# proycon/analiticcl

Hardware: AMD Instinct MI355X
Metric: scored (query,candidate) pairs/sec + queries/sec, 200k-lexicon, len≤16, 1/2/4/8 GPU (higher is better)
Workload: dtype u8

## Files before the change

analiticcl_amd/_lib.py:

```python
from __future__ import annotations

import ctypes as C
import os

HERE = os.path.dirname(os.path.abspath(__file__))
LIB_PATH = os.environ.get("ANX_LIB") or os.path.join(HERE, "libanx.so")

ANX_OK, ANX_EINVAL, ANX_EIO, ANX_ENOTBUILT, ANX_ENODEVICE, ANX_ELIMIT, ANX_EEMPTY = 0, -1, -2, -3, -4, -5, -6
ANX_NO_VIA = 0xFFFFFFFFFFFFFFFF
ABI_VERSION = 3


class AnxError(RuntimeError):
    def __init__(self, code: int, message: str):
        super().__init__(f"anx error {code}: {message}")
        self.code = code


class Weights(C.Structure):
    _fields_ = [("ld", C.c_double), ("lcs", C.c_double), ("prefix", C.c_double), ("suffix", C.c_double),
                ("casew", C.c_double)]


class Threshold(C.Structure):
# ... 185 lines not shown
        "anx_shutdown": (None, []),
        "anx_pipeline_new": (vp, [vp, C.c_int]),
        "anx_pipeline_submit_packed": (C.c_int, [vp, cp, C.c_size_t, C.c_size_t, C.POINTER(Params)]),
        "anx_pipeline_pending": (C.c_int, [vp]),
        "anx_pipeline_next": (C.c_int, [vp, C.POINTER(vp), C.POINTER(C.POINTER(C.c_uint32)), C.POINTER(C.c_size_t)]),
        "anx_pipeline_next_via": (C.c_int, [vp, C.POINTER(vp), C.POINTER(C.POINTER(C.c_uint32)), C.POINTER(C.POINTER(C.c_uint32)), C.POINTER(C.c_size_t)]),
        "anx_pipeline_free": (None, [vp]),
        "anx_debug_kernel_timer": (None, [C.c_int]),
        "anx_debug_kernel_time": (C.c_int, [cp, C.POINTER(C.c_double), C.POINTER(C.c_uint64)]),
        "anx_debug_length_split": (C.c_int, [vp, C.POINTER(C.c_char_p), C.c_size_t, C.POINTER(Params), C.c_int, vp, vp]),
        "anx_debug_signature": (C.c_int, [vp, cp, C.POINTER(C.c_uint64)]),
        "anx_debug_entries": (C.c_int, [vp, C.POINTER(C.POINTER(C.c_uint32)), C.POINTER(C.c_size_t)]),
        "anx_debug_adjacency": (C.c_int, [vp, C.c_int, C.c_uint64, vp, C.c_size_t, vp, C.POINTER(C.POINTER(C.c_uint32)), vp]),
        "anx_debug_adjacency_device": (C.c_int, [vp, vp, C.c_size_t, vp, C.POINTER(C.POINTER(C.c_uint32))]),
        "anx_debug_band_bound": (C.c_int, [C.c_int, vp, vp, vp, vp, C.c_size_t, C.c_int, C.c_int, vp]),
        "anx_batch_free": (None, [vp]),
        "anx_device_pool_trim": (None, [C.c_int]),
    }
    for name, (res, args) in sig.items():
        fn = getattr(L, name)
        fn.restype = res
        fn.argtypes = args
    _lib = L
    return L


EXPORTED = None


def set_switch(name: str, value) -> None:
# ... 21 lines not shown
```

analiticcl_amd/csrc/engine.h:

```cpp
#pragma once
#include <cstdint>
#include <string>
#include <vector>

#include "host_model.h"
#include "adjacency.h"

namespace anx {

struct DeviceLexicon;
struct Batch;

int device_count(std::string& err);
DeviceLexicon* lexicon_upload(const LexiconImage& img, const EncodeTables& et, const AdjIndex* adj, int device, std::string& err, int dev_closure = -1,
                              size_t dev_budget = 0, AdjIndex* dev_stats = nullptr);
void lexicon_free(DeviceLexicon*);
int debug_band_bound(int device, const uint8_t* q_rows, const uint8_t* c_rows, const uint8_t* lq, const uint8_t* lc, size_t n, int d, int form,
                     uint8_t* out, std::string& err);
void kernel_timer_enable(bool on);
bool kernel_timer_read(const char* name, double* total_ms, uint64_t* launches);
void device_pool_trim(int device);
void* stream_create(int device, std::string& err, bool high_priority = false);
void stream_destroy(int device, void* stream);
void* host_result_alloc(size_t bytes);
bool host_result_is_pinned(void* p);
void host_result_free(void* p);
void* thread_stream_begin(int device);
void thread_stream_end(int device, void* stream);
void encoder_stream_set_override(void* stream);
void host_result_cache_stats(uint64_t* hits, uint64_t* misses, uint64_t* miss_bytes);

Batch* batch_encode(const HostModel& m, const DeviceLexicon* dl, const char* const* utf8, size_t n,
                    const anx_params& p, std::string& err, int* code, bool keep_text = false);
// ... 124 lines not shown
```

analiticcl_amd/csrc/engine.hip:

```cpp
#include <hip/hip_runtime.h>

#include <algorithm>
#include <atomic>
#include <functional>
#include <chrono>
#include <cmath>
#include <cstdio>
#include <cstdlib>
#include <cstring>
#include <map>
#include <memory>
#include <mutex>
#include <unordered_map>
#include <numeric>
#include <thread>
#include <type_traits>

#include "engine_internal.h"

namespace anx {

#define HIP_TRY(expr)                                                                          \
  do {                                                                                         \
    hipError_t _e = (expr);                                                                    \
// ... 882 lines not shown
static void shells_destroy(int device) {
  DevPool& pl = pool_of(device);
  std::vector<BatchShell> drop;
  { std::lock_guard<std::mutex> g(pl.mu); drop.swap(pl.shells); }
  for (BatchShell& sh : drop) {
    for (auto& e : sh.ev) if (e) (void)hipEventDestroy(e);
    for (hipEvent_t e : {sh.ev_fs0, sh.ev_fs1, sh.ev_scan0, sh.ev_done, sh.ev_in}) if (e) (void)hipEventDestroy(e);
    if (sh.h_read) (void)hipHostFree(sh.h_read);
  }
}

static int encode_tail(Batch* b, std::string& err) {
  const size_t nq = b->nq;
  int rc;
  const size_t nblk = (nq + SCAN_TILE - 1) / SCAN_TILE + 2;
  if ((rc = dalloc(&b->counters, CTR_N, err)) || (rc = dalloc(&b->rctr, SCAN_REGIONS * RC_STRIDE, err)) || (rc = dalloc(&b->sctr, SCAN_REGIONS * RC_STRIDE, err)) || (rc = dalloc(&b->lctr, 3 * SCAN_REGIONS * RC_STRIDE, err)) || (rc = dalloc(&b->qexpand, nq, err)) || (rc = dalloc(&b->qsurv, nq, err)) ||
      (rc = dalloc(&b->soff, nq + 1, err)) || (rc = dalloc(&b->qcur, nq, err)) || (rc = dalloc(&b->qmaxfreq, nq, err)) ||
      (rc = dalloc(&b->scan_tmp, nblk, err)) || (rc = dalloc(&b->r_count, nq, err)) || (rc = dalloc(&b->r_off, nq + 1, err)))
    return rc;
  return shell_acquire(b, err);
}

Batch* batch_encode_spans(const HostModel& m, const DeviceLexicon* dl, const char* blob, size_t blob_bytes, const uint32_t* off, size_t n,
                          const anx_params& p, std::string& err, int* code, bool keep_text, bool blob_on_device, bool after_stream, void* src_stream) {
  *code = ANX_OK;
  if (blob_on_device && (off || switches().encode_host)) { err = "inputs in device memory need the device-side encoder and no host offsets"; *code = ANX_EINVAL; return nullptr; }
  if (!dl) { err = "model is not resident on a device (no HIP device / anx_model_to_device not called)"; *code = ANX_ENODEVICE; return nullptr; }
  if (hipSetDevice(dl->device) != hipSuccess) { err = "hipSetDevice failed"; *code = ANX_ENODEVICE; return nullptr; }
  if (n >= (1u << 27)) { err = "more than 2^27 inputs per batch"; *code = ANX_ELIMIT; return nullptr; }
  Batch* b = new Batch();
  b->device = dl->device;
  b->params = p;
  b->n_input = n;
  b->keep_text = keep_text;
// ... 54 lines not shown
  HostBuf<char> blob(part[nthreads] + 1);
  if (!blob.data()) { err = "out of memory"; *code = ANX_ELIMIT; return nullptr; }
  run_threads([&](unsigned t, size_t lo, size_t hi) {
    size_t pos = part[t];
    for (size_t i = lo; i < hi; ++i) {
      off[i] = (uint32_t)pos;
      if (lens[i]) memcpy(&blob[pos], utf8[i], lens[i]);
      blob[pos + lens[i]] = '\0';
      pos += (size_t)lens[i] + 1;
    }
  });
  off[n] = (uint32_t)part[nthreads];
  return batch_encode_spans(m, dl, blob.data(), blob.size(), off.data(), n, p, err, code, keep_text);
}

static int exclusive_scan(const uint32_t* in, uint32_t n, uint32_t* out, uint32_t* tmp, hipStream_t st, uint32_t* maxout = nullptr, uint32_t* copy = nullptr) {
  const uint32_t nb = (n + SCAN_TILE - 1) / SCAN_TILE;
  if (nb == 0) return hipMemsetAsync(out, 0, sizeof(uint32_t), st) == hipSuccess ? 0 : -1;
  hipLaunchKernelGGL(k_scan_local, dim3(nb), dim3(SCAN_THREADS), 0, st, in, n, out, tmp, maxout);
  hipLaunchKernelGGL(k_scan_sums, dim3(1), dim3(SCAN_THREADS), 0, st, tmp, nb);
  hipLaunchKernelGGL(k_scan_add, dim3(nb), dim3(SCAN_THREADS), 0, st, out, n, tmp, nb, copy);
  return 0;
}

namespace {
struct KTimerRec { std::string name; hipEvent_t e0 = nullptr, e1 = nullptr; int device = 0; bool closed = false; };
struct KTimer {
  std::mutex mu;
  std::atomic<bool> on{false};
  std::vector<KTimerRec> pending;
  uint32_t generation = 0;
  std::map<std::string, std::pair<double, uint64_t>> acc;
};
KTimer& ktimer() { static KTimer* t = new KTimer; return *t; }
void ktimer_resolve_locked(KTimer& t) {
  for (KTimerRec& r : t.pending) {
// ... 210 lines not shown
int Run::setup() {
  int rc;
  hints_apply(dl, b);
  if (b->raw_cap == 0 && b->hinted && (rc = ensure_raw(b, (size_t)b->prev_maxfill + (b->prev_maxfill >> 3) + 4096, err))) return rc;
  if (b->raw_cap == 0 && (rc = ensure_raw(b, (nq * (size_t)140 + (size_t)b->ntiles * SCAN_CHUNK) / SCAN_REGIONS / cap_div() + 4096, err)))
    return rc;
  region_cap = 1u << b->region_shift;
  fill_cap = b->prev_maxfill ? (uint32_t)std::min<size_t>(region_cap, (size_t)b->prev_maxfill + (b->prev_maxfill >> 3) + FS_BLK) : region_cap;
  b->fill_cap_launched = fill_cap;
  HIP_TRY(hipEventRecord(b->ev[0], st));
  return ANX_OK;
}

int Run::scan() {
  int rc;
  HIP_TRY(hipMemsetAsync(b->counters, 0, CTR_N * sizeof(uint32_t), st));
  HIP_TRY(hipMemsetAsync(b->rctr, 0, SCAN_REGIONS * RC_STRIDE * sizeof(uint32_t), st));
  if (b->ntiles == 0) { HIP_TRY(hipEventRecord(b->ev_scan0, st)); HIP_TRY(hipEventRecord(b->ev[5], st)); }
  if (b->ntiles) {
    ScanArgs A = scan_args_of(dl);
    A.tiles = b->d_tiles; A.ntiles = b->ntiles; A.q_bits = b->q_bits; A.q_cv = b->q_cv;
    A.chunk = SCAN_CHUNK;
    A.chunk_fused = switches().scan_chunk_fused ? (uint32_t)switches().scan_chunk_fused : SCAN_CHUNK_FUSED;
#ifdef ANX_DEBUG_SWITCHES
    { const char* e = getenv("ANX_SCAN_CHUNK"); const int v = e ? atoi(e) : 0; if (v >= 32 && v <= 1024) A.chunk = (uint32_t)v; }
#endif
    A.raw = b->raw; A.region_cap = region_cap; A.rctr = b->rctr; A.qexact = b->qexact; A.want_exact = stop;
    A.drop_len = (!stop && !b->keep_all_pairs) ? 1 : 0;
    A.q_rec = b->q_rec;
    A.fuse = (switches().fuse_prefilter && switches().prefilter && A.drop_len) ? 1 : 0;
    A.qpairs = nullptr;
    if (b->count_pairs) {
      if (!b->qpairs && (rc = dalloc(&b->qpairs, nq, err))) return rc;
      HIP_TRY(hipMemsetAsync(b->qpairs, 0, nq * sizeof(uint32_t), st));
      A.qpairs = b->qpairs;
    }
    A.dbg = 0;
#ifdef ANX_DEBUG_SWITCHES
    { const char* e = getenv("ANX_SCAN_DBG"); A.dbg = e ? atoi(e) : 0; }
#endif
    const uint32_t nsad = b->n_sad_tiles, nbits = A.ntiles - nsad, nadj = std::min(b->n_adj_tiles, nbits);
    with_nplanes(dl->nplanes, [&](auto np) { launch_scan<decltype(np)::value>(A, nadj, nbits, nsad, st, b->ev_scan0, b->ev[5]); });
  }
  HIP_TRY(hipMemcpyAsync(b->h_read + HR_RCTR, b->rctr, SCAN_REGIONS * RC_STRIDE * sizeof(uint32_t), hipMemcpyDeviceToHost, st));
  HIP_TRY(hipEventRecord(b->ev[1], st));
  b->n_raw = (uint32_t)(SCAN_REGIONS << b->region_shift);
  return ANX_OK;
}

int Run::score() {
  int rc;
  HIP_TRY(hipMemsetAsync(b->qsurv, 0, nq * sizeof(uint32_t), st));
  HIP_TRY(hipMemsetAsync(b->qmaxfreq, 0, nq * sizeof(uint32_t), st));
  if (dl->any_variants) HIP_TRY(hipMemsetAsync(b->qexpand, 0, nq * sizeof(uint32_t), st));
  ScorePlan plan = score_plan_of(m, dl, b->params.score_threshold, b->qw, b->dmax);
  ScoreArgs& sa = plan.sa;
#ifdef ANX_DEBUG_SWITCHES
  { const char* e = getenv("ANX_SCORE_DBG"); sa.dbg = e ? atoi(e) : 0; }
#endif
  sa.store_pairs = b->keep_all_pairs ? 1 : 0;
  if (sa.store_pairs && (rc = ensure_pair_outputs(b, err))) return rc;
  if (!plan.fits()) { err = "per-lane scoring state exceeds the LDS budget"; return ANX_ELIMIT; }
  const int fastD = plan.fastD;
  if ((rc = ensure_surv_records(b, b->prev_surv_fill ? (size_t)b->prev_surv_fill + (b->prev_surv_fill >> 3) + 256 : (size_t)fill_cap / 2 / cap_div() + 256, err))) return rc;
  so = SurvOut{b->surv, b->sctr, (uint32_t)b->surv_region_cap, nullptr, seg_capacity(dl, b)};
  so.seg = so.seg_cap ? b->sseg : nullptr;
  const bool need_lists = !fastD || plan.have_long_q || dl->max_len > 16;
  if (need_lists && (rc = ensure_slot_lists(b, b->prev_list_fill ? (size_t)b->prev_list_fill + (b->prev_list_fill >> 3) + 256 : (fastD ? (size_t)fill_cap / 2 : (size_t)fill_cap) / cap_div() + 256, err)))
    return rc;
  HIP_TRY(hipMemsetAsync(b->sctr, 0, SCAN_REGIONS * RC_STRIDE * sizeof(uint32_t), st));
  HIP_TRY(hipMemsetAsync(b->lctr, 0, 3 * SCAN_REGIONS * RC_STRIDE * sizeof(uint32_t), st));
  const SlotLists sl = slot_lists_of(b->list8, b->listg, b->listw, b->lctr, (uint32_t)b->list_cap);
  const PairArgs pa = pair_args_of(dl, b->raw, b->q_meta, b->q_rows, b->q_rec, b->p_score, b->p_meta, b->qmaxfreq, b->qsurv, b->qexpand);
  FilterArgs fa;
  fa.region_shift = b->region_shift; fa.rctr = b->rctr; fa.qexact = b->qexact; fa.stop = stop; fa.enable = plan.enable_filter;
  fa.use_nw8 = (plan.have_long_q || fastD > 0) ? 1 : 0; fa.counters = b->counters; fa.stat_ctr = b->sctr; fa.fill_cap = fill_cap; fa.blk = FS_BLK;
  const dim3 fgrid(((fill_cap + FS_BLK - 1) / FS_BLK) * SCAN_REGIONS);
  {
    FsCold* cold = reinterpret_cast<FsCold*>(reinterpret_cast<char*>(b->h_read) + HR_COLD_OFF);
    *cold = FsCold{sa, so, sl.l8, sl.lg, sl.lw};
    if (!b->d_cold && (rc = dalloc(reinterpret_cast<char**>(&b->d_cold), sizeof(FsCold), err))) return rc;
    HIP_TRY(hipMemcpyAsync(b->d_cold, cold, sizeof(FsCold), hipMemcpyHostToDevice, st));
  }
  HIP_TRY(hipEventRecord(b->ev_fs0, st));
  launch_filter_score(plan, fgrid, st, fa, pa, static_cast<const FsCold*>(b->d_cold));
  HIP_TRY(hipEventRecord(b->ev_fs1, st));
  if (need_lists) {
    const dim3 lgrid(LIST_P * SCAN_REGIONS);
    if (plan.split_wide && plan.enable_filter) hipLaunchKernelGGL(k_filter_wide, lgrid, dim3(256), 0, st, sl.lw, fa, pa, sa, fastD, sl.l8, sl.lg);
    if (fastD) launch_score_fast8(fastD, lgrid, st, sl.l8, pa, sa, so);
    hipLaunchKernelGGL(k_score_pairs, lgrid, dim3(plan.threads), plan.lds_bytes(), st, sl.lg, pa, sa, so);
  }
  HIP_TRY(hipEventRecord(b->ev[2], st));
  return ANX_OK;
}

int Run::compact_rank() {
  int rc;
  const RankArgs ra = rank_args_of(m, dl, b->params, b->conf_mode == 1 ? 0.0 : b->params.cutoff_threshold);
  exclusive_scan(b->qsurv, nq, b->soff, b->scan_tmp, st, nullptr, b->qcur);
  if (dl->any_variants) {
    uint32_t total_surv = 0;
    HIP_TRY(hipMemcpyAsync(&total_surv, b->soff + nq, sizeof(uint32_t), hipMemcpyDeviceToHost, st));
    HIP_TRY(hipMemcpyAsync(b->h_read + HR_SCTR, b->sctr, SCAN_REGIONS * RC_STRIDE * sizeof(uint32_t), hipMemcpyDeviceToHost, st));
    HIP_TRY(hipStreamSynchronize(st));
    uint32_t surv_fill = 0;
    for (uint32_t r = 0; r < SCAN_REGIONS; ++r) surv_fill = std::max(surv_fill, b->h_read[HR_SCTR + r * RC_STRIDE]);
    if ((size_t)surv_fill > b->surv_region_cap) {
      surv_fill = 0;
      HIP_TRY(hipMemsetAsync(b->counters + CTR_OVERFLOW, 0xFF, sizeof(uint32_t), st));
    }
    if ((rc = ensure_surv(b, (size_t)total_surv + (total_surv >> 2) + 1024, err))) return rc;
    if (surv_fill) {
      CompactArgs ca{m.have_freq ? 1 : 0, dl->any_variants};
      hipLaunchKernelGGL(k_compact, dim3(((surv_fill + 255) / 256) * SCAN_REGIONS), dim3(256), 0, st, b->surv, b->sctr,
                         (uint32_t)b->surv_region_cap, ca, b->qcur, dl->ent_rec, dl->ent_var_off, dl->var_target,
                         dl->var_target_freq, dl->var_score, b->c_rows);
    }
  } else if (b->surv_cap == 0 && (rc = ensure_surv(b, b->hint_rows ? b->hint_rows : (size_t)nq * 16 / cap_div() + 1024, err))) return rc;
  const uint32_t row_cap = (uint32_t)std::min<size_t>(b->surv_cap, 0xFFFFFFFFu);
  if (!dl->any_variants)
    hipLaunchKernelGGL(k_compact_grouped, dim3(COMPACT_P * SCAN_REGIONS), dim3(COMPACT_B), 0, st, b->surv, b->sctr,
                       (uint32_t)b->surv_region_cap, m.have_freq ? 1 : 0, b->qcur, dl->ent_rec, b->c_rows, b->soff + nq, row_cap,
                       b->counters + CTR_OVERFLOW);
  HIP_TRY(hipEventRecord(b->ev[3], st));
  if (b->conf_mode == 2 && (rc = conf_launch(m, dl, b, st, true, row_cap, err))) return rc;
  launch_rank(ra, st, nq, b->soff, b->c_rows, b->qmaxfreq, b->qexpand, b->t_key, b->r_rows, b->r_count, dl->any_variants ? 0xFFFFFFFFu : row_cap, b->counters + CTR_OVERFLOW,
              dl->any_variants ? SegRows{nullptr, 0u, nullptr} : SegRows{so.seg, so.seg_cap, dl->ent_rec});
  if (b->conf_mode == 1 && (rc = conf_launch(m, dl, b, st, false, row_cap, err))) return rc;
  exclusive_scan(b->r_count, nq, b->r_off, b->scan_tmp, st, b->counters + CTR_MAXROWS);
  HIP_TRY(hipEventRecord(b->ev[4], st));
  return ANX_OK;
}

int Run::readback() {
  HIP_TRY(hipMemcpyAsync(b->h_read + HR_SCTR, b->sctr, SCAN_REGIONS * RC_STRIDE * sizeof(uint32_t), hipMemcpyDeviceToHost, st));
  HIP_TRY(hipMemcpyAsync(b->h_read + HR_LCTR, b->lctr, 3 * SCAN_REGIONS * RC_STRIDE * sizeof(uint32_t), hipMemcpyDeviceToHost, st));
  HIP_TRY(hipMemcpyAsync(b->h_read + HR_CTR, b->counters, CTR_N * sizeof(uint32_t), hipMemcpyDeviceToHost, st));
  HIP_TRY(hipMemcpyAsync(b->h_read + HR_TOTAL_SURV, b->soff + nq, sizeof(uint32_t), hipMemcpyDeviceToHost, st));
  HIP_TRY(hipMemcpyAsync(b->h_read + HR_TOTAL_RESULTS, b->r_off + nq, sizeof(uint32_t), hipMemcpyDeviceToHost, st));
  b->h_read[HR_CONF] = b->h_read[HR_CONF + 1] = 0;
  if (b->conf_mode && b->cf_ctr) HIP_TRY(hipMemcpyAsync(b->h_read + HR_CONF, b->cf_ctr, 2 * sizeof(uint32_t), hipMemcpyDeviceToHost, st));
  HIP_TRY(hipEventRecord(b->ev_done, st));
  HIP_TRY(hipGetLastError());
  return ANX_OK;
}

static int batch_launch(const HostModel& m, const DeviceLexicon* dl, Batch* b, void* stream, std::string& err) {
  if (!dl) { err = "model is not resident on a device"; return ANX_ENODEVICE; }
  if (b->nq >= (1u << 27) || dl->nentries >= (1u << 26)) { err = "more than 2^27 queries per batch or 2^26 lexicon entries (32-bit record offsets, packed pair records)"; return ANX_ELIMIT; }
  HIP_TRY(hipSetDevice(dl->device));
  if (b->launched) {
    HIP_TRY(hipEventSynchronize(b->ev_done));
    b->launched = false;
  }
  b->last_stream = stream;
  b->ran = false;
// ... 431 lines not shown
  HIP_TRY(hipSetDevice(b->device));
  off.assign(b->n_input + 1, 0u);
  HIP_TRY(hipMemcpy(off.data(), b->d_textoff, (b->n_input + 1) * sizeof(uint32_t), hipMemcpyDeviceToHost));
  text.assign(b->n_input ? (size_t)off[b->n_input] : 0, '\0');
  if (!text.empty()) HIP_TRY(hipMemcpy(&text[0], b->d_text, text.size(), hipMemcpyDeviceToHost));
  return ANX_OK;
}

void batch_stats(const Batch* b, anx_batch_stats* s) { *s = b->stats; }

void batch_free(Batch* b) {
  if (!b) return;
  (void)hipSetDevice(b->device);
  if (b->async_pending) (void)hipStreamSynchronize(reinterpret_cast<hipStream_t>(b->async_stream));
  if (b->launched) (void)hipEventSynchronize(b->ev_done);
  for (void* p : {(void*)b->q_cv, (void*)b->q_bits, (void*)b->q_rows, (void*)b->q_rec, (void*)b->q_meta, (void*)b->q_orig, (void*)b->d_tiles, (void*)b->rctr, (void*)b->sctr, (void*)b->surv,
                  (void*)b->counters, (void*)b->qexact, (void*)b->qsurv, (void*)b->soff, (void*)b->qcur,
                  (void*)b->qmaxfreq, (void*)b->d_cold, (void*)b->qpairs, (void*)b->x_cnt, (void*)b->x_tmp, (void*)b->scan_tmp, (void*)b->raw, (void*)b->p_score, (void*)b->p_meta, (void*)b->list8, (void*)b->listg, (void*)b->listw, (void*)b->lctr,
                  (void*)b->c_rows, (void*)b->sseg, (void*)b->qexpand, (void*)b->r_rows, (void*)b->t_key, (void*)b->r_count, (void*)b->r_off,
                  (void*)b->d_text, (void*)b->d_textoff, (void*)b->cf_weight, (void*)b->cf_need, (void*)b->cf_ctr, b->cf_work, (void*)b->cf_sort, b->cf_sort_tmp})
    if (p) pool_free(p);
  shell_release(b);
  delete b;
}

#include "small_path.hpp"

__global__ __launch_bounds__(64) void k_debug_band_bound(const uint4* __restrict__ q, const uint4* __restrict__ c, const uint8_t* __restrict__ lqs,
                                                         const uint8_t* __restrict__ lcs, uint32_t n, int d, int form, uint8_t* __restrict__ out) {
  const uint32_t i = blockIdx.x * 64u + threadIdx.x;
  const bool act = i < n;
  const uint4 Q = act ? q[i] : make_uint4(0xFEFEFEFEu, 0xFEFEFEFEu, 0xFEFEFEFEu, 0xFEFEFEFEu);
  const uint4 C = act ? c[i] : make_uint4(0xFFFFFFFFu, 0xFFFFFFFFu, 0xFFFFFFFFu, 0xFFFFFFFFu);
  const int lq = act ? lqs[i] : 1, lc = act ? lcs[i] : 1;
// ... 33 lines not shown
  auto fail_hip = [&](hipError_t e) { err = std::string("HIP: ") + hipGetErrorString(e); cleanup(); return ANX_ENODEVICE; };
  hipError_t e;
  if ((e = hipMalloc(reinterpret_cast<void**>(&dq), n * 16)) != hipSuccess || (e = hipMalloc(reinterpret_cast<void**>(&dc), n * 16)) != hipSuccess ||
      (e = hipMalloc(reinterpret_cast<void**>(&dlq), n)) != hipSuccess || (e = hipMalloc(reinterpret_cast<void**>(&dlc), n)) != hipSuccess ||
      (e = hipMalloc(reinterpret_cast<void**>(&dout), n)) != hipSuccess)
    return fail_hip(e);
  if ((e = hipMemcpy(dq, q_rows, n * 16, hipMemcpyHostToDevice)) != hipSuccess || (e = hipMemcpy(dc, c_rows, n * 16, hipMemcpyHostToDevice)) != hipSuccess ||
      (e = hipMemcpy(dlq, lq, n, hipMemcpyHostToDevice)) != hipSuccess || (e = hipMemcpy(dlc, lc, n, hipMemcpyHostToDevice)) != hipSuccess)
    return fail_hip(e);
  hipLaunchKernelGGL(k_debug_band_bound, dim3((uint32_t)((n + 63) / 64)), dim3(64), 0, 0, dq, dc, dlq, dlc, (uint32_t)n, d, form, dout);
  if ((e = hipDeviceSynchronize()) != hipSuccess || (e = hipMemcpy(out, dout, n, hipMemcpyDeviceToHost)) != hipSuccess) return fail_hip(e);
  cleanup();
  return rc;
}

}
```

analiticcl_amd/csrc/export_capi.cpp:

```cpp
#include <functional>
#include <string>
#include <vector>

#include "engine.h"
#include "host_model.h"

size_t anx_export_num_shards(const anx_batch* b);
void anx_export_shard(const anx_batch* b, size_t g, void* caller_stream, const anx::DeviceLexicon** dl, anx::Batch** sb, void** stream);
int anx_export_on_shards(const anx_batch* b, const std::function<int(size_t, std::string&)>& fn);
bool anx_batch_host_rescored(const anx_batch* b);
int anx_fail(int code, const std::string& msg);

namespace {
struct ShardRef {
  const anx::DeviceLexicon* dl = nullptr;
  anx::Batch* b = nullptr;
  void* stream = nullptr;
};
ShardRef shard_of(const anx_batch* b, size_t g, void* caller_stream) {
  ShardRef s;
  anx_export_shard(b, g, caller_stream, &s.dl, &s.b, &s.stream);
  return s;
}
int check_export(const anx_batch* b) {
  if (!b) return anx_fail(ANX_EINVAL, "NULL batch");
  if (anx_batch_host_rescored(b)) return anx_fail(ANX_EINVAL, "confusables are loaded: results are rescored on the host, use anx_batch_fetch");
  if (anx_export_num_shards(b) != 1) return anx_fail(ANX_EINVAL, "the batch is spread over several replicas: export one shard at a time (anx_batch_shard_*)");
  return ANX_OK;
}
}

extern "C" {
int anx_batch_export_topk_via(const anx_batch* b, void* dst, void* via, uint32_t stride, void* stream) {
  if (int rc = check_export(b)) return rc;
  const ShardRef s = shard_of(b, 0, stream);
  if (!s.b) return anx_fail(ANX_EINVAL, "batch has not been run");
  std::string err;
  const int rc = anx::batch_export_topk_via(s.dl, s.b, dst, via, stride, stream, err);
  return rc ? anx_fail(rc, err) : ANX_OK;
}
int anx_batch_export_compact_via(const anx_batch* b, void* dst, size_t capacity, void* stream, size_t* used) {
  if (!used) return anx_fail(ANX_EINVAL, "NULL argument");
  if (int rc = check_export(b)) return rc;
  const ShardRef s = shard_of(b, 0, stream);
  if (!s.b) return anx_fail(ANX_EINVAL, "batch has not been run");
  std::string err;
  const int rc = anx::batch_export_compact_via(s.dl, s.b, dst, capacity, stream, used, err);
// ... 23 lines not shown
```

analiticcl_amd/csrc/kernels_common.hpp:

```cpp
#pragma once

struct Tile {
  uint32_t q0, nq;
  uint32_t s0, s1;
  uint32_t k;
  uint32_t lq;
  uint32_t sig_lo, sig_hi;
  uint32_t kind;
  uint32_t d;
  uint32_t kend;
  uint32_t ball0, balln;
  uint32_t adj;
  uint32_t flags;
};
constexpr uint32_t BALL_MAX = 4096;
constexpr uint32_t SIG_BYTE_MAX = 120;

constexpr int kSymbolPlanesMaxA = 61;
__host__ __device__ inline void symbol_planes16(const uint8_t* row, uint32_t len, uint32_t (&w)[3]) {
  uint32_t p[6] = {0u, 0u, 0u, 0u, 0u, 0u};
  for (uint32_t i = 0; i < 16u && i < len; ++i) {
    const uint32_t v = (uint32_t)row[i] + 1u;
    for (uint32_t b = 0; b < 6u; ++b) p[b] |= ((v >> b) & 1u) << i;
  }
// ... 125 lines not shown
  std::vector<Tile> tiles;
  uint32_t ntiles = 0;
  uint32_t n_sad_tiles = 0;
  uint32_t n_adj_tiles = 0;
  uint32_t qw = 1;
  uint32_t dmax = 0;
  uint64_t n_class_tests = 0;
  uint64_t n_tests_kind[NBITPLANES + 1] = {};
  uint32_t* q_cv = nullptr;
  uint32_t* q_bits = nullptr;
  uint4* q_rows = nullptr;
  uint4* q_rec = nullptr;
  uint32_t* q_meta = nullptr;
  uint32_t* q_orig = nullptr;
  Tile* d_tiles = nullptr;
  uint32_t* counters = nullptr;
  uint32_t* rctr = nullptr;
  uint32_t region_shift = 0;
  uint32_t region_fill[SCAN_REGIONS] = {};
  uint32_t* qexact = nullptr;
  uint32_t* qsurv = nullptr;
  uint32_t* soff = nullptr;
  uint32_t* qcur = nullptr;
  uint32_t* qmaxfreq = nullptr;
  void* d_cold = nullptr;
  uint32_t* qpairs = nullptr;
  bool count_pairs = false;
  int conf_mode = 0;
  bool keep_text = false;
  uint8_t* d_text = nullptr;
// ... 19 lines not shown
  uint32_t* listw = nullptr;
  uint32_t* lctr = nullptr;
  size_t list_cap = 0;
  size_t raw_cap = 0;
  SurvRec* surv = nullptr;
  uint32_t* sctr = nullptr;
  size_t surv_region_cap = 0;
  SurvRow* c_rows = nullptr;
  SurvSeg* sseg = nullptr;
  size_t sseg_cap = 0;
  uint32_t* qexpand = nullptr;
  DevRow* r_rows = nullptr;
  double* t_key = nullptr;
  size_t surv_cap = 0;
  uint32_t* r_count = nullptr;
  uint32_t* r_off = nullptr;
  uint32_t n_raw = 0;
  uint64_t n_sel = 0;
  uint64_t n_pairs = 0, n_surv = 0, n_results = 0;
  mutable uint32_t *x_cnt = nullptr, *x_tmp = nullptr;
  uint32_t max_rows = 0;
  void* last_stream = nullptr;
  mutable void* async_stream = nullptr;
  mutable bool async_pending = false;
  bool ran = false;
  bool keep_all_pairs = false;
  bool ran_keep_all = false;
  hipEvent_t ev[6] = {};
  hipEvent_t ev_scan0 = nullptr;
  hipEvent_t ev_fs0 = nullptr, ev_fs1 = nullptr;
  hipEvent_t ev_done = nullptr;
// ... 20 lines not shown
```

analiticcl_amd/csrc/kernels_prefix.hpp:

```cpp
#pragma once

constexpr int SCAN_ITEMS = 8, SCAN_THREADS = 256, SCAN_TILE = SCAN_ITEMS * SCAN_THREADS;

__device__ inline uint32_t block_exclusive_scan(uint32_t v, uint32_t* total) {
  __shared__ uint32_t wsum[SCAN_THREADS / 64];
  const int lane = threadIdx.x & 63, wid = threadIdx.x >> 6;
  uint32_t inc = v;
#pragma unroll
  for (int o = 1; o < 64; o <<= 1) {
    const uint32_t u = __shfl_up(inc, o);
    if (lane >= o) inc += u;
  }
  if (lane == 63) wsum[wid] = inc;
  __syncthreads();
  uint32_t base = 0, tot = 0;
  for (int i = 0; i < SCAN_THREADS / 64; ++i) {
    if (i < wid) base += wsum[i];
    tot += wsum[i];
  }
  __syncthreads();
  *total = tot;
  return base + inc - v;
}
__global__ __launch_bounds__(SCAN_THREADS) void k_scan_local(const uint32_t* __restrict__ in, uint32_t n,
                                                             uint32_t* __restrict__ out,
                                                             uint32_t* __restrict__ blocksum, uint32_t* __restrict__ maxout) {
  const uint32_t i0 = blockIdx.x * SCAN_TILE + threadIdx.x * SCAN_ITEMS;
  uint32_t v[SCAN_ITEMS], s = 0;
#pragma unroll
  for (int i = 0; i < SCAN_ITEMS; ++i) {
    v[i] = i0 + i < n ? in[i0 + i] : 0;
    s += v[i];
  }
  uint32_t tot;
  uint32_t ex = block_exclusive_scan(s, &tot);
#pragma unroll
  for (int i = 0; i < SCAN_ITEMS; ++i) {
    if (i0 + i < n) out[i0 + i] = ex;
    ex += v[i];
  }
  if (threadIdx.x == 0) blocksum[blockIdx.x] = tot;
  if (maxout) {
    uint32_t mx = 0;
#pragma unroll
    for (int i = 0; i < SCAN_ITEMS; ++i) mx = max(mx, v[i]);
#pragma unroll
    for (int o = 32; o; o >>= 1) mx = max(mx, (uint32_t)__shfl_xor((int)mx, o));
    if ((threadIdx.x & 63) == 0 && mx) atomicMax(maxout, mx);
  }
}
__global__ __launch_bounds__(SCAN_THREADS) void k_scan_sums(uint32_t* __restrict__ blocksum, uint32_t nb) {
  uint32_t carry = 0;
  for (uint32_t b0 = 0; b0 < nb; b0 += SCAN_THREADS) {
    const uint32_t i = b0 + threadIdx.x;
    const uint32_t v = i < nb ? blocksum[i] : 0;
    uint32_t tot;
    const uint32_t ex = block_exclusive_scan(v, &tot);
    if (i < nb) blocksum[i] = carry + ex;
    carry += tot;
  }
  if (threadIdx.x == 0) blocksum[nb] = carry;
}
__global__ __launch_bounds__(SCAN_THREADS) void k_scan_add(uint32_t* __restrict__ out, uint32_t n,
                                                           const uint32_t* __restrict__ blocksum, uint32_t nb, uint32_t* __restrict__ copy) {
  const uint32_t i0 = blockIdx.x * SCAN_TILE + threadIdx.x * SCAN_ITEMS;
  const uint32_t add = blocksum[blockIdx.x];
#pragma unroll
  for (int i = 0; i < SCAN_ITEMS; ++i)
    if (i0 + i < n) {
      const uint32_t v = out[i0 + i] + add;
      out[i0 + i] = v;
      if (copy) copy[i0 + i] = v;
    }
  if (blockIdx.x == 0 && threadIdx.x == 0) out[n] = blocksum[nb];
}
```

analiticcl_amd/csrc/kernels_rank.hpp:

```cpp
#pragma once

struct CompactArgs {
  int have_freq, any_variants;
};
__global__ __launch_bounds__(256) void k_compact(const SurvRec* __restrict__ surv, const uint32_t* __restrict__ sctr,
                                                 uint32_t region_cap, CompactArgs a,
                                                 uint32_t* __restrict__ qcur, const EntRec* __restrict__ ent_rec,
                                                 const uint32_t* __restrict__ ent_var_off,
                                                 const uint32_t* __restrict__ var_target,
                                                 const uint32_t* __restrict__ var_target_freq,
                                                 const double* __restrict__ var_score, SurvRow* __restrict__ c_rows) {
  const uint32_t region = blockIdx.x % SCAN_REGIONS, i = (blockIdx.x / SCAN_REGIONS) * 256 + threadIdx.x;
  const bool live = i < sctr[region * RC_STRIDE];
  if (!live) return;
  const SurvRec sr = surv[(size_t)region * region_cap + i];
  const double s = sr.score;
  const uint32_t e = sr.e, q = sr.q;
  const EntRec er = ent_rec[e];
  const uint32_t f = a.have_freq ? er.freq : 1u;
  const unsigned long long ord = (unsigned long long)er.order << 20;
  uint32_t v0 = 0, v1 = 0, self = 1;
  if (a.any_variants) {
    v0 = ent_var_off[e];
    v1 = ent_var_off[e + 1];
// ... 553 lines not shown
    for (int k = 0; k < RANK_QPW; ++k) {
      if (qbase + k >= nq) break;
      const uint32_t nk = (uint32_t)__builtin_amdgcn_readlane((int)my_n, k);
      if (nk <= 32u) continue;
      rank_query<64, RANK_LCAP>(qbase + k, true, lane, 0, nk, reinterpret_cast<double*>(wl),
                                reinterpret_cast<unsigned long long*>(wl + RANK_LCAP * 8),
                                reinterpret_cast<uint32_t*>(wl + RANK_LCAP * 16), reinterpret_cast<uint16_t*>(wl + RANK_LCAP * 20),
                                reinterpret_cast<double*>(wl + RANK_LCAP * 22), reinterpret_cast<double*>(wl + RANK_LCAP * 22 + 512),
                                (uint32_t)__shfl((int)my_seg0, k), nk, (uint32_t)__shfl((int)my_maxf, k), (uint32_t)__shfl((int)my_qex, k),
                                c_rows, sr, a, t_key, r_rows, r_count);
      __builtin_amdgcn_fence(__ATOMIC_SEQ_CST, "workgroup");
    }
  }
}

__global__ __launch_bounds__(256) void k_pack_rows(uint32_t nq, const uint32_t* __restrict__ soff,
                                                   const uint32_t* __restrict__ r_off,
                                                   const uint32_t* __restrict__ r_count,
                                                   const DevRow* __restrict__ r_rows, DevRow* __restrict__ out) {
  const uint32_t q = blockIdx.x * 256 + threadIdx.x;
  if (q >= nq) return;
  const uint32_t n = r_count[q], src = soff[q], dst = r_off[q];
  for (uint32_t i = 0; i < n; ++i) out[dst + i] = r_rows[src + i];
}
__global__ __launch_bounds__(256) void k_fetch_counts(uint32_t nq, const uint32_t* __restrict__ r_count,
                                                      const uint32_t* __restrict__ q_orig, uint32_t* __restrict__ cnt_orig) {
  const uint32_t s = blockIdx.x * 256 + threadIdx.x;
  if (s < nq) cnt_orig[q_orig[s]] = r_count[s];
}
__device__ inline anx_topk_record topk_record_of(const DevRow& d) {
  anx_topk_record r;
  r.vocab_id = d.vocab_id;
  r.freq_score = (float)d.freq_score;
  r.dist_score = d.dist_score;
  return r;
}
struct EmitResult {
  anx_result* out;
  __device__ void operator()(uint32_t at, const DevRow& d) const {
// ... 153 lines not shown
```

include/anx.h:

```cpp
#ifndef ANX_H
#define ANX_H
#include <stddef.h>
#include <stdint.h>
#ifdef __cplusplus
extern "C" {
#endif

#define ANX_ABI_VERSION 3

enum {
  ANX_OK = 0,
  ANX_EINVAL = -1,
  ANX_EIO = -2,
  ANX_ENOTBUILT = -3,
  ANX_ENODEVICE = -4,
  ANX_ELIMIT = -5,
  ANX_EEMPTY = -6
};

typedef struct anx_model anx_model;
typedef struct anx_batch anx_batch;

typedef struct anx_weights {
  double ld, lcs, prefix, suffix, casew;
// ... 172 lines not shown
int anx_debug_search_stats(uint64_t out[4]);
int anx_debug_search_lattice_stats(uint64_t out[4]);
int anx_debug_contextrule_match(const anx_model *model, size_t rule, size_t position, uint64_t vocab_id, uint32_t lexindex, int flat, int *out);
int anx_debug_small_stats(uint64_t out[2]);
int anx_debug_small_conf_stats(uint64_t out[3]);
int anx_debug_small_replica_stats(const anx_model *model, uint64_t *out, size_t cap);
int anx_debug_length_split(const anx_model *, const char *const *utf8, size_t n, const anx_params *, int n_shards, uint8_t *out_shard,
                           const double *learn_ms);
int anx_debug_signature(const anx_model *, const char *utf8, uint64_t *out_sig);
int anx_debug_entries(const anx_model *, uint32_t **out_vocab_ids, size_t *n);
int anx_debug_adjacency(const anx_model *, int closure, uint64_t budget_bytes, const uint64_t *sigs, size_t n, uint32_t *out_cum,
                        uint32_t **out_ids, uint64_t *out_stats);
int anx_debug_adjacency_device(const anx_model *, const uint64_t *sigs, size_t n, uint32_t *out_cum, uint32_t **out_ids);
int anx_debug_band_bound(int device, const uint8_t *q_rows, const uint8_t *c_rows, const uint8_t *lq, const uint8_t *lc, size_t n,
                         int d, int form, uint8_t *out_reject);

int anx_format_query_output(const anx_model *, const char *const *utf8_inputs, size_t n, const anx_result *rows,
                            const size_t *offsets, float freq_weight, int json, int output_lexmatch,
                            uint64_t first_seqnr, char **out, size_t *out_len);
void anx_string_free(char *);

int anx_model_add_to_confusables(anx_model *, const char *editscript, double weight);
int anx_model_read_confusablelist(anx_model *, const char *path);
void anx_model_set_confusables_before_pruning(anx_model *);
int anx_edit_script(const char *source, const char *target, char *out, int cap);
int anx_model_confusable_weight(const anx_model *, const char *input_utf8, uint64_t vocab_id, double *out_weight);

typedef struct anx_search_params {
  anx_params base;
  uint8_t max_ngram;
// ... 51 lines not shown
```

Measured before the change: 55.95 billion.

## Consolidate batch control counters and trim scan/readback launches per run

```diff
diff --git a/analiticcl_amd/_lib.py b/analiticcl_amd/_lib.py
--- a/analiticcl_amd/_lib.py
+++ b/analiticcl_amd/_lib.py
@@ -223,6 +223,7 @@
         "anx_debug_adjacency": (C.c_int, [vp, C.c_int, C.c_uint64, vp, C.c_size_t, vp, C.POINTER(C.POINTER(C.c_uint32)), vp]),
         "anx_debug_adjacency_device": (C.c_int, [vp, vp, C.c_size_t, vp, C.POINTER(C.POINTER(C.c_uint32))]),
         "anx_debug_band_bound": (C.c_int, [C.c_int, vp, vp, vp, vp, C.c_size_t, C.c_int, C.c_int, vp]),
+        "anx_debug_exclusive_scan": (C.c_int, [C.c_int, vp, C.c_size_t, vp, vp]),
         "anx_batch_free": (None, [vp]),
         "anx_device_pool_trim": (None, [C.c_int]),
     }
diff --git a/analiticcl_amd/csrc/engine.h b/analiticcl_amd/csrc/engine.h
--- a/analiticcl_amd/csrc/engine.h
+++ b/analiticcl_amd/csrc/engine.h
@@ -17,6 +17,7 @@
 void lexicon_free(DeviceLexicon*);
 int debug_band_bound(int device, const uint8_t* q_rows, const uint8_t* c_rows, const uint8_t* lq, const uint8_t* lc, size_t n, int d, int form,
                      uint8_t* out, std::string& err);
+int debug_exclusive_scan(int device, const uint32_t* in, size_t n, uint32_t* out, uint32_t* copy, std::string& err);
 void kernel_timer_enable(bool on);
 bool kernel_timer_read(const char* name, double* total_ms, uint64_t* launches);
 void device_pool_trim(int device);
diff --git a/analiticcl_amd/csrc/engine.hip b/analiticcl_amd/csrc/engine.hip
--- a/analiticcl_amd/csrc/engine.hip
+++ b/analiticcl_amd/csrc/engine.hip
@@ -920,10 +920,12 @@
   const size_t nq = b->nq;
   int rc;
   const size_t nblk = (nq + SCAN_TILE - 1) / SCAN_TILE + 2;
-  if ((rc = dalloc(&b->counters, CTR_N, err)) || (rc = dalloc(&b->rctr, SCAN_REGIONS * RC_STRIDE, err)) || (rc = dalloc(&b->sctr, SCAN_REGIONS * RC_STRIDE, err)) || (rc = dalloc(&b->lctr, 3 * SCAN_REGIONS * RC_STRIDE, err)) || (rc = dalloc(&b->qexpand, nq, err)) || (rc = dalloc(&b->qsurv, nq, err)) ||
-      (rc = dalloc(&b->soff, nq + 1, err)) || (rc = dalloc(&b->qcur, nq, err)) || (rc = dalloc(&b->qmaxfreq, nq, err)) ||
-      (rc = dalloc(&b->scan_tmp, nblk, err)) || (rc = dalloc(&b->r_count, nq, err)) || (rc = dalloc(&b->r_off, nq + 1, err)))
+  if ((rc = dalloc(&b->ctl, HR_N, err)) || (rc = dalloc(&b->qsurv, 3 * nq, err)) ||
+      (rc = dalloc(&b->soff, nq + 1, err)) || (rc = dalloc(&b->qcur, nq, err)) ||
+      (rc = dalloc(&b->scan_tmp, nblk, err)) || (rc = dalloc(&b->r_count, nq, err)))
     return rc;
+  b->rctr = b->ctl + HR_RCTR; b->sctr = b->ctl + HR_SCTR; b->lctr = b->ctl + HR_LCTR; b->counters = b->ctl + HR_CTR;
+  b->qmaxfreq = b->qsurv + nq; b->qexpand = b->qsurv + 2 * nq;
   return shell_acquire(b, err);
 }
 
@@ -1008,12 +1010,13 @@
   return batch_encode_spans(m, dl, blob.data(), blob.size(), off.data(), n, p, err, code, keep_text);
 }
 
-static int exclusive_scan(const uint32_t* in, uint32_t n, uint32_t* out, uint32_t* tmp, hipStream_t st, uint32_t* maxout = nullptr, uint32_t* copy = nullptr) {
+static int exclusive_scan(const uint32_t* in, uint32_t n, uint32_t* out, uint32_t* tmp, hipStream_t st, uint32_t* copy = nullptr) {
   const uint32_t nb = (n + SCAN_TILE - 1) / SCAN_TILE;
   if (nb == 0) return hipMemsetAsync(out, 0, sizeof(uint32_t), st) == hipSuccess ? 0 : -1;
-  hipLaunchKernelGGL(k_scan_local, dim3(nb), dim3(SCAN_THREADS), 0, st, in, n, out, tmp, maxout);
-  hipLaunchKernelGGL(k_scan_sums, dim3(1), dim3(SCAN_THREADS), 0, st, tmp, nb);
-  hipLaunchKernelGGL(k_scan_add, dim3(nb), dim3(SCAN_THREADS), 0, st, out, n, tmp, nb, copy);
+  const int fused = nb <= SCAN_FUSED_BLOCKS ? 1 : 0;
+  hipLaunchKernelGGL(k_scan_local, dim3(nb), dim3(SCAN_THREADS), 0, st, in, n, out, tmp);
+  if (!fused) hipLaunchKernelGGL(k_scan_sums, dim3(1), dim3(SCAN_THREADS), 0, st, tmp, nb);
+  hipLaunchKernelGGL(k_scan_add, dim3(nb), dim3(SCAN_THREADS), 0, st, out, n, tmp, nb, copy, fused);
   return 0;
 }
 
@@ -1254,8 +1257,7 @@
 
 int Run::scan() {
   int rc;
-  HIP_TRY(hipMemsetAsync(b->counters, 0, CTR_N * sizeof(uint32_t), st));
-  HIP_TRY(hipMemsetAsync(b->rctr, 0, SCAN_REGIONS * RC_STRIDE * sizeof(uint32_t), st));
+  HIP_TRY(hipMemsetAsync(b->ctl, 0, HR_N * sizeof(uint32_t), st));
   if (b->ntiles == 0) { HIP_TRY(hipEventRecord(b->ev_scan0, st)); HIP_TRY(hipEventRecord(b->ev[5], st)); }
   if (b->ntiles) {
     ScanArgs A = scan_args_of(dl);
@@ -1282,7 +1284,6 @@
     const uint32_t nsad = b->n_sad_tiles, nbits = A.ntiles - nsad, nadj = std::min(b->n_adj_tiles, nbits);
     with_nplanes(dl->nplanes, [&](auto np) { launch_scan<decltype(np)::value>(A, nadj, nbits, nsad, st, b->ev_scan0, b->ev[5]); });
   }
-  HIP_TRY(hipMemcpyAsync(b->h_read + HR_RCTR, b->rctr, SCAN_REGIONS * RC_STRIDE * sizeof(uint32_t), hipMemcpyDeviceToHost, st));
   HIP_TRY(hipEventRecord(b->ev[1], st));
   b->n_raw = (uint32_t)(SCAN_REGIONS << b->region_shift);
   return ANX_OK;
@@ -1290,9 +1291,7 @@
 
 int Run::score() {
   int rc;
-  HIP_TRY(hipMemsetAsync(b->qsurv, 0, nq * sizeof(uint32_t), st));
-  HIP_TRY(hipMemsetAsync(b->qmaxfreq, 0, nq * sizeof(uint32_t), st));
-  if (dl->any_variants) HIP_TRY(hipMemsetAsync(b->qexpand, 0, nq * sizeof(uint32_t), st));
+  HIP_TRY(hipMemsetAsync(b->qsurv, 0, (dl->any_variants ? 3 : 2) * (size_t)nq * sizeof(uint32_t), st));
   ScorePlan plan = score_plan_of(m, dl, b->params.score_threshold, b->qw, b->dmax);
   ScoreArgs& sa = plan.sa;
 #ifdef ANX_DEBUG_SWITCHES
@@ -1308,8 +1307,6 @@
   const bool need_lists = !fastD || plan.have_long_q || dl->max_len > 16;
   if (need_lists && (rc = ensure_slot_lists(b, b->prev_list_fill ? (size_t)b->prev_list_fill + (b->prev_list_fill >> 3) + 256 : (fastD ? (size_t)fill_cap / 2 : (size_t)fill_cap) / cap_div() + 256, err)))
     return rc;
-  HIP_TRY(hipMemsetAsync(b->sctr, 0, SCAN_REGIONS * RC_STRIDE * sizeof(uint32_t), st));
-  HIP_TRY(hipMemsetAsync(b->lctr, 0, 3 * SCAN_REGIONS * RC_STRIDE * sizeof(uint32_t), st));
   const SlotLists sl = slot_lists_of(b->list8, b->listg, b->listw, b->lctr, (uint32_t)b->list_cap);
   const PairArgs pa = pair_args_of(dl, b->raw, b->q_meta, b->q_rows, b->q_rec, b->p_score, b->p_meta, b->qmaxfreq, b->qsurv, b->qexpand);
   FilterArgs fa;
@@ -1338,7 +1335,7 @@
 int Run::compact_rank() {
   int rc;
   const RankArgs ra = rank_args_of(m, dl, b->params, b->conf_mode == 1 ? 0.0 : b->params.cutoff_threshold);
-  exclusive_scan(b->qsurv, nq, b->soff, b->scan_tmp, st, nullptr, b->qcur);
+  exclusive_scan(b->qsurv, nq, b->soff, b->scan_tmp, st, b->qcur);
   if (dl->any_variants) {
     uint32_t total_surv = 0;
     HIP_TRY(hipMemcpyAsync(&total_surv, b->soff + nq, sizeof(uint32_t), hipMemcpyDeviceToHost, st));
@@ -1368,19 +1365,15 @@
   launch_rank(ra, st, nq, b->soff, b->c_rows, b->qmaxfreq, b->qexpand, b->t_key, b->r_rows, b->r_count, dl->any_variants ? 0xFFFFFFFFu : row_cap, b->counters + CTR_OVERFLOW,
               dl->any_variants ? SegRows{nullptr, 0u, nullptr} : SegRows{so.seg, so.seg_cap, dl->ent_rec});
   if (b->conf_mode == 1 && (rc = conf_launch(m, dl, b, st, false, row_cap, err))) return rc;
-  exclusive_scan(b->r_count, nq, b->r_off, b->scan_tmp, st, b->counters + CTR_MAXROWS);
+  hipLaunchKernelGGL(k_run_summary, dim3((nq + SCAN_THREADS * SUMMARY_ITEMS - 1) / (SCAN_THREADS * SUMMARY_ITEMS)), dim3(SCAN_THREADS), 0, st, b->r_count, nq, b->ctl,
+                     (uint32_t)HR_TOTAL_RESULTS, (uint32_t)(HR_CTR + CTR_MAXROWS), b->soff + nq, (uint32_t)HR_TOTAL_SURV,
+                     (b->conf_mode && b->cf_ctr) ? b->cf_ctr : nullptr, (uint32_t)HR_CONF);
   HIP_TRY(hipEventRecord(b->ev[4], st));
   return ANX_OK;
 }
 
 int Run::readback() {
-  HIP_TRY(hipMemcpyAsync(b->h_read + HR_SCTR, b->sctr, SCAN_REGIONS * RC_STRIDE * sizeof(uint32_t), hipMemcpyDeviceToHost, st));
-  HIP_TRY(hipMemcpyAsync(b->h_read + HR_LCTR, b->lctr, 3 * SCAN_REGIONS * RC_STRIDE * sizeof(uint32_t), hipMemcpyDeviceToHost, st));
-  HIP_TRY(hipMemcpyAsync(b->h_read + HR_CTR, b->counters, CTR_N * sizeof(uint32_t), hipMemcpyDeviceToHost, st));
-  HIP_TRY(hipMemcpyAsync(b->h_read + HR_TOTAL_SURV, b->soff + nq, sizeof(uint32_t), hipMemcpyDeviceToHost, st));
-  HIP_TRY(hipMemcpyAsync(b->h_read + HR_TOTAL_RESULTS, b->r_off + nq, sizeof(uint32_t), hipMemcpyDeviceToHost, st));
-  b->h_read[HR_CONF] = b->h_read[HR_CONF + 1] = 0;
-  if (b->conf_mode && b->cf_ctr) HIP_TRY(hipMemcpyAsync(b->h_read + HR_CONF, b->cf_ctr, 2 * sizeof(uint32_t), hipMemcpyDeviceToHost, st));
+  HIP_TRY(hipMemcpyAsync(b->h_read, b->ctl, HR_N * sizeof(uint32_t), hipMemcpyDeviceToHost, st));
   HIP_TRY(hipEventRecord(b->ev_done, st));
   HIP_TRY(hipGetLastError());
   return ANX_OK;
@@ -1842,10 +1835,10 @@
   (void)hipSetDevice(b->device);
   if (b->async_pending) (void)hipStreamSynchronize(reinterpret_cast<hipStream_t>(b->async_stream));
   if (b->launched) (void)hipEventSynchronize(b->ev_done);
-  for (void* p : {(void*)b->q_cv, (void*)b->q_bits, (void*)b->q_rows, (void*)b->q_rec, (void*)b->q_meta, (void*)b->q_orig, (void*)b->d_tiles, (void*)b->rctr, (void*)b->sctr, (void*)b->surv,
-                  (void*)b->counters, (void*)b->qexact, (void*)b->qsurv, (void*)b->soff, (void*)b->qcur,
-                  (void*)b->qmaxfreq, (void*)b->d_cold, (void*)b->qpairs, (void*)b->x_cnt, (void*)b->x_tmp, (void*)b->scan_tmp, (void*)b->raw, (void*)b->p_score, (void*)b->p_meta, (void*)b->list8, (void*)b->listg, (void*)b->listw, (void*)b->lctr,
-                  (void*)b->c_rows, (void*)b->sseg, (void*)b->qexpand, (void*)b->r_rows, (void*)b->t_key, (void*)b->r_count, (void*)b->r_off,
+  for (void* p : {(void*)b->q_cv, (void*)b->q_bits, (void*)b->q_rows, (void*)b->q_rec, (void*)b->q_meta, (void*)b->q_orig, (void*)b->d_tiles, (void*)b->ctl, (void*)b->surv,
+                  (void*)b->qexact, (void*)b->qsurv, (void*)b->soff, (void*)b->qcur,
+                  (void*)b->d_cold, (void*)b->qpairs, (void*)b->x_cnt, (void*)b->x_tmp, (void*)b->scan_tmp, (void*)b->raw, (void*)b->p_score, (void*)b->p_meta, (void*)b->list8, (void*)b->listg, (void*)b->listw,
+                  (void*)b->c_rows, (void*)b->sseg, (void*)b->r_rows, (void*)b->t_key, (void*)b->r_count,
                   (void*)b->d_text, (void*)b->d_textoff, (void*)b->cf_weight, (void*)b->cf_need, (void*)b->cf_ctr, b->cf_work, (void*)b->cf_sort, b->cf_sort_tmp})
     if (p) pool_free(p);
   shell_release(b);
@@ -1909,4 +1902,23 @@
   return rc;
 }
 
-}
+int debug_exclusive_scan(int device, const uint32_t* in, size_t n, uint32_t* out, uint32_t* copy, std::string& err) {
+  if (n >= ((size_t)1 << 31)) { err = "prefix sum: more than 2^31 elements"; return ANX_EINVAL; }
+  HIP_TRY(hipSetDevice(device));
+  uint32_t *din = nullptr, *dout = nullptr, *dcopy = nullptr, *dtmp = nullptr;
+  auto cleanup = [&]() { for (void* p : {(void*)din, (void*)dout, (void*)dcopy, (void*)dtmp}) if (p) (void)hipFree(p); };
+  auto fail_hip = [&](hipError_t e) { err = std::string("HIP: ") + hipGetErrorString(e); cleanup(); return ANX_ENODEVICE; };
+  hipError_t e;
+  if ((e = hipMalloc(reinterpret_cast<void**>(&din), (n + 1) * 4)) != hipSuccess || (e = hipMalloc(reinterpret_cast<void**>(&dout), (n + 1) * 4)) != hipSuccess ||
+      (e = hipMalloc(reinterpret_cast<void**>(&dcopy), (n + 1) * 4)) != hipSuccess || (e = hipMalloc(reinterpret_cast<void**>(&dtmp), scan_tmp_bytes(n))) != hipSuccess)
+    return fail_hip(e);
+  if (n && (e = hipMemcpy(din, in, n * 4, hipMemcpyHostToDevice)) != hipSuccess) return fail_hip(e);
+  if (exclusive_scan(din, (uint32_t)n, dout, dtmp, 0, copy ? dcopy : nullptr)) return fail_hip(hipGetLastError());
+  if ((e = hipDeviceSynchronize()) != hipSuccess || (e = hipMemcpy(out, dout, (n + 1) * 4, hipMemcpyDeviceToHost)) != hipSuccess ||
+      (copy && n && (e = hipMemcpy(copy, dcopy, n * 4, hipMemcpyDeviceToHost)) != hipSuccess))
+    return fail_hip(e);
+  cleanup();
+  return ANX_OK;
+}
+
+}
diff --git a/analiticcl_amd/csrc/export_capi.cpp b/analiticcl_amd/csrc/export_capi.cpp
--- a/analiticcl_amd/csrc/export_capi.cpp
+++ b/analiticcl_amd/csrc/export_capi.cpp
@@ -31,6 +31,12 @@
 }
 
 extern "C" {
+int anx_debug_exclusive_scan(int device, const uint32_t* in, size_t n, uint32_t* out, uint32_t* copy) {
+  if (!out || (!in && n)) return anx_fail(ANX_EINVAL, "NULL argument");
+  std::string err;
+  const int rc = anx::debug_exclusive_scan(device, in, n, out, copy, err);
+  return rc ? anx_fail(rc, err) : ANX_OK;
+}
 int anx_batch_export_topk_via(const anx_batch* b, void* dst, void* via, uint32_t stride, void* stream) {
   if (int rc = check_export(b)) return rc;
   const ShardRef s = shard_of(b, 0, stream);
diff --git a/analiticcl_amd/csrc/kernels_common.hpp b/analiticcl_amd/csrc/kernels_common.hpp
--- a/analiticcl_amd/csrc/kernels_common.hpp
+++ b/analiticcl_amd/csrc/kernels_common.hpp
@@ -163,6 +163,7 @@
   uint32_t* q_meta = nullptr;
   uint32_t* q_orig = nullptr;
   Tile* d_tiles = nullptr;
+  uint32_t* ctl = nullptr;
   uint32_t* counters = nullptr;
   uint32_t* rctr = nullptr;
   uint32_t region_shift = 0;
@@ -212,7 +213,6 @@
   double* t_key = nullptr;
   size_t surv_cap = 0;
   uint32_t* r_count = nullptr;
-  uint32_t* r_off = nullptr;
   uint32_t n_raw = 0;
   uint64_t n_sel = 0;
   uint64_t n_pairs = 0, n_surv = 0, n_results = 0;
diff --git a/analiticcl_amd/csrc/kernels_prefix.hpp b/analiticcl_amd/csrc/kernels_prefix.hpp
--- a/analiticcl_amd/csrc/kernels_prefix.hpp
+++ b/analiticcl_amd/csrc/kernels_prefix.hpp
@@ -24,7 +24,7 @@
 }
 __global__ __launch_bounds__(SCAN_THREADS) void k_scan_local(const uint32_t* __restrict__ in, uint32_t n,
                                                              uint32_t* __restrict__ out,
-                                                             uint32_t* __restrict__ blocksum, uint32_t* __restrict__ maxout) {
+                                                             uint32_t* __restrict__ blocksum) {
   const uint32_t i0 = blockIdx.x * SCAN_TILE + threadIdx.x * SCAN_ITEMS;
   uint32_t v[SCAN_ITEMS], s = 0;
 #pragma unroll
@@ -40,14 +40,6 @@
     ex += v[i];
   }
   if (threadIdx.x == 0) blocksum[blockIdx.x] = tot;
-  if (maxout) {
-    uint32_t mx = 0;
-#pragma unroll
-    for (int i = 0; i < SCAN_ITEMS; ++i) mx = max(mx, v[i]);
-#pragma unroll
-    for (int o = 32; o; o >>= 1) mx = max(mx, (uint32_t)__shfl_xor((int)mx, o));
-    if ((threadIdx.x & 63) == 0 && mx) atomicMax(maxout, mx);
-  }
 }
 __global__ __launch_bounds__(SCAN_THREADS) void k_scan_sums(uint32_t* __restrict__ blocksum, uint32_t nb) {
   uint32_t carry = 0;
@@ -61,10 +53,33 @@
   }
   if (threadIdx.x == 0) blocksum[nb] = carry;
 }
+__device__ inline uint32_t block_sum(uint32_t v) {
+  __shared__ uint32_t wsum[SCAN_THREADS / 64];
+#pragma unroll
+  for (int o = 32; o; o >>= 1) v += (uint32_t)__shfl_xor((int)v, o);
+  if ((threadIdx.x & 63) == 0) wsum[threadIdx.x >> 6] = v;
+  __syncthreads();
+  uint32_t tot = 0;
+#pragma unroll
+  for (int i = 0; i < SCAN_THREADS / 64; ++i) tot += wsum[i];
+  return tot;
+}
+constexpr uint32_t SCAN_FUSED_BLOCKS = 1024;
 __global__ __launch_bounds__(SCAN_THREADS) void k_scan_add(uint32_t* __restrict__ out, uint32_t n,
-                                                           const uint32_t* __restrict__ blocksum, uint32_t nb, uint32_t* __restrict__ copy) {
+                                                           const uint32_t* __restrict__ blocksum, uint32_t nb, uint32_t* __restrict__ copy, int fused) {
   const uint32_t i0 = blockIdx.x * SCAN_TILE + threadIdx.x * SCAN_ITEMS;
-  const uint32_t add = blocksum[blockIdx.x];
+  uint32_t add, total;
+  if (fused) {
+    const uint32_t lim = blockIdx.x ? blockIdx.x : nb;
+    uint32_t s = 0;
+    for (uint32_t i = threadIdx.x; i < lim; i += SCAN_THREADS) s += blocksum[i];
+    s = block_sum(s);
+    add = blockIdx.x ? s : 0u;
+    total = s;
+  } else {
+    add = blocksum[blockIdx.x];
+    total = blockIdx.x ? 0u : blocksum[nb];
+  }
 #pragma unroll
   for (int i = 0; i < SCAN_ITEMS; ++i)
     if (i0 + i < n) {
@@ -72,5 +87,35 @@
       out[i0 + i] = v;
       if (copy) copy[i0 + i] = v;
     }
-  if (blockIdx.x == 0 && threadIdx.x == 0) out[n] = blocksum[nb];
+  if (blockIdx.x == 0 && threadIdx.x == 0) out[n] = total;
 }
+
+constexpr int SUMMARY_ITEMS = 16;
+__global__ __launch_bounds__(SCAN_THREADS) void k_run_summary(const uint32_t* __restrict__ r_count, uint32_t nq, uint32_t* __restrict__ ctl,
+                                                              uint32_t w_total, uint32_t w_max, const uint32_t* __restrict__ soff_end, uint32_t w_surv,
+                                                              const uint32_t* __restrict__ cf_ctr, uint32_t w_conf) {
+  __shared__ uint32_t wmax[SCAN_THREADS / 64];
+  uint32_t s = 0, mx = 0;
+  const uint32_t base = blockIdx.x * (SCAN_THREADS * SUMMARY_ITEMS) + threadIdx.x;
+#pragma unroll 4
+  for (int i = 0; i < SUMMARY_ITEMS; ++i) {
+    const uint32_t q = base + i * SCAN_THREADS;
+    const uint32_t v = q < nq ? r_count[q] : 0u;
+    s += v;
+    mx = max(mx, v);
+  }
+#pragma unroll
+  for (int o = 32; o; o >>= 1) mx = max(mx, (uint32_t)__shfl_xor((int)mx, o));
+  if ((threadIdx.x & 63) == 0) wmax[threadIdx.x >> 6] = mx;
+  s = block_sum(s);
+  if (threadIdx.x == 0) {
+#pragma unroll
+    for (int i = 0; i < SCAN_THREADS / 64; ++i) mx = max(mx, wmax[i]);
+    if (s) atomicAdd(ctl + w_total, s);
+    if (mx) atomicMax(ctl + w_max, mx);
+    if (blockIdx.x == 0) {
+      ctl[w_surv] = *soff_end;
+      if (cf_ctr) { ctl[w_conf] = cf_ctr[0]; ctl[w_conf + 1] = cf_ctr[1]; }
+    }
+  }
+}
diff --git a/analiticcl_amd/csrc/kernels_rank.hpp b/analiticcl_amd/csrc/kernels_rank.hpp
--- a/analiticcl_amd/csrc/kernels_rank.hpp
+++ b/analiticcl_amd/csrc/kernels_rank.hpp
@@ -591,15 +591,6 @@
   }
 }
 
-__global__ __launch_bounds__(256) void k_pack_rows(uint32_t nq, const uint32_t* __restrict__ soff,
-                                                   const uint32_t* __restrict__ r_off,
-                                                   const uint32_t* __restrict__ r_count,
-                                                   const DevRow* __restrict__ r_rows, DevRow* __restrict__ out) {
-  const uint32_t q = blockIdx.x * 256 + threadIdx.x;
-  if (q >= nq) return;
-  const uint32_t n = r_count[q], src = soff[q], dst = r_off[q];
-  for (uint32_t i = 0; i < n; ++i) out[dst + i] = r_rows[src + i];
-}
 __global__ __launch_bounds__(256) void k_fetch_counts(uint32_t nq, const uint32_t* __restrict__ r_count,
                                                       const uint32_t* __restrict__ q_orig, uint32_t* __restrict__ cnt_orig) {
   const uint32_t s = blockIdx.x * 256 + threadIdx.x;
diff --git a/include/anx.h b/include/anx.h
--- a/include/anx.h
+++ b/include/anx.h
@@ -210,6 +210,7 @@
 int anx_debug_adjacency_device(const anx_model *, const uint64_t *sigs, size_t n, uint32_t *out_cum, uint32_t **out_ids);
 int anx_debug_band_bound(int device, const uint8_t *q_rows, const uint8_t *c_rows, const uint8_t *lq, const uint8_t *lc, size_t n,
                          int d, int form, uint8_t *out_reject);
+int anx_debug_exclusive_scan(int device, const uint32_t *in, size_t n, uint32_t *out, uint32_t *copy);
 
 int anx_format_query_output(const anx_model *, const char *const *utf8_inputs, size_t n, const anx_result *rows,
                             const size_t *offsets, float freq_weight, int json, int output_lexmatch,
```

Measured after the change: 56.64 billion, median of 6. +1.2%, better.
